# yg838457845/ORB_SLAM2-Chinese-annotation

Measured on AMD Instinct MI355X. Metric: frames/sec (extract+match) at 1241×376, 1000 feat/frame; 1/2/4/8 GPU, higher is better.
Workload: dtype u8; 1 GPU; C4: 1241x376 KITTI-shaped synthetic stream, 1000 feat/frame, SearchByProjection vs 5000-point local map per frame; distinct_frames_per_gpu=8192, frames_per_launch=1024, parallelism=single rank; no collective (one process, one GPU)

## Files before the change

### orb_slam2-chinese-annotation_amd/csrc/extractor_kernels.hip

```cpp
#include <stdlib.h>
#include <type_traits>
#include <algorithm>
#include "orb_device.h"
#include "orb_plan.h"
#include "orb_kernels.h"
#include "orb_pattern_data.h"
#include "../../include/orb_abi.h"

#define PYR_TW 128
#ifndef PYR_IMAGES_PER_WG
#define PYR_IMAGES_PER_WG 16
#endif
#define PYR_TH 32
#define PYR_SROWS 44
#define PYR_SW 44
#define PYR_SROWS_WIDE 64
#define PYR_SW_WIDE 64

__global__ __launch_bounds__(256) void k_pyr_resize_generic(
    const uint8_t* __restrict__ src, long long srcImgPitch, int srcStride, int sw, int sh,
    uint8_t* __restrict__ dst, long long dstImgPitch, int dstStride, int dw, int dh,
    const int* __restrict__ xofs, const int* __restrict__ alpha, const int* __restrict__ yofs,
    const int* __restrict__ beta) {
  const int xs = 4 * (blockIdx.x * 64 + (int)(threadIdx.x & 63));
// ... 789 lines not shown
  h16x2 w3[16];
#pragma unroll
  for (int k = 0; k < 16; ++k)
    w3[k] = __builtin_bit_cast(h16x2, pk_min3_negpair(r[k], r[(k + 1) & 15], r[(k + 2) & 15]));
  h16x2 w9[16];
#pragma unroll
  for (int k = 0; k < 16; ++k)
    w9[k] = __builtin_elementwise_minimum(__builtin_elementwise_minimum(w3[k], w3[(k + 3) & 15]),
                                          w3[(k + 6) & 15]);
  h16x2 m5[6];
#pragma unroll
  for (int k = 0; k < 5; ++k)
    m5[k] = __builtin_elementwise_maximum(__builtin_elementwise_maximum(w9[3 * k], w9[3 * k + 1]),
                                          w9[3 * k + 2]);
  m5[5] = w9[15];
  const h16x2 ma = __builtin_elementwise_maximum(__builtin_elementwise_maximum(m5[0], m5[1]), m5[2]);
  const h16x2 mb = __builtin_elementwise_maximum(__builtin_elementwise_maximum(m5[3], m5[4]), m5[5]);
  h16x2 best = __builtin_elementwise_maximum(ma, mb);
  const _Float16 v = __builtin_bit_cast(_Float16, (uint16_t)c[0]);
  const h16x2 vv = {v, -v};
  best = best + vv;
  const int s = (int)(short)__builtin_bit_cast(uint16_t, __builtin_fmaxf16(best.x, best.y));
  return min(max(s, 0), 255);
}

#ifndef FC_WPE
#define FC_WPE 7
#endif
template <int PT>
__global__ __launch_bounds__(64 * FC_WAVES) __attribute__((amdgpu_waves_per_eu(FC_WPE)))
void k_fast_cells(
    const uint8_t* __restrict__ img0, long long img0Pitch, int img0Stride,
    const uint8_t* __restrict__ arena, long long arenaPitch, OrbPlanDesc plan,
    const OrbCellDesc* __restrict__ cells, uint32_t* __restrict__ cellKeys,
    int32_t* __restrict__ cellCount, int tileElems, int cellBeg, int cellEnd,
    int32_t* __restrict__ errFlag) {
  extern __shared__ __attribute__((aligned(16))) unsigned char smem[];
  const int lane = threadIdx.x & 63;
  const int wave = __builtin_amdgcn_readfirstlane(threadIdx.x >> 6);
  int bx, img;
  xcd_swizzle(bx, img);
  if (errFlag && bx == 0 && threadIdx.x == 0) errFlag[img] = 0;
  uint8_t* tile = smem + wave * fc_wave_bytes(tileElems);
  uint8_t* sc = tile + tileElems;
  uint16_t* queue = (uint16_t*)(sc + tileElems);
  uint16_t* corners = queue + FC_QCAP;
  auto cell_of = [&](int j) { return cellBeg + (bx * FC_CPW + j) * FC_WAVES + wave; };
  uint32_t raw[16], rsh = 0;
  auto issue = [&](const OrbCellDesc& q) {
    const int ql = q.level, qR = q.y1 - q.y0;
    const uint8_t* lvl;
    int pitch;
    if (ql == 0) {
      lvl = img0 + (long long)img * img0Pitch;
      pitch = img0Stride;
    } else {
      lvl = arena + (long long)img * arenaPitch + plan.lv[ql].arenaOff;
      pitch = plan.lv[ql].pitch;
    }
    const ImgRsrc im = img_rsrc(lvl, (uint32_t)((plan.lv[ql].h - 1) * pitch + plan.lv[ql].w));
    const int r = min(lane, max(qR - 1, 0));
    const uint32_t o = (uint32_t)((q.y0 + r) * pitch + q.x0 - FAST_LPAD) + im.sh;
    rsh = o & 3u;
    const uint32_t a0 = o & ~3u;
#pragma unroll
    for (int k = 0; k < 4; ++k) {
      const auto v = __builtin_amdgcn_raw_buffer_load_b128(im.r, (int)(a0 + 16 * k), 0, 0);
      raw[4 * k] = (uint32_t)v[0];
      raw[4 * k + 1] = (uint32_t)v[1];
      raw[4 * k + 2] = (uint32_t)v[2];
      raw[4 * k + 3] = (uint32_t)v[3];
    }
  };
  int ci = cell_of(0);
  if (ci >= cellEnd) return;
  OrbCellDesc ncd = cells[ci];
  issue(ncd);
  for (int jc = 0; jc < FC_CPW && ci < cellEnd; ++jc) {
  const OrbCellDesc cd = ncd;
  const int R = cd.y1 - cd.y0, C = cd.x1 - cd.x0;
  const long long slot = (long long)img * plan.ncells + ci;
  const bool tiny = R < 7 || C < 7;
  const int P = PT ? PT : fc_pitch(C);
  if (!tiny && lane < R) {
    const int nS = P >> 2;
    uint2* dst = reinterpret_cast<uint2*>(tile + lane * P);
#pragma unroll
    for (int k = 0; k < 7; ++k) {
      if (2 * k < nS)
        dst[k] = make_uint2(__builtin_amdgcn_alignbyte(raw[2 * k + 1], raw[2 * k], rsh),
                            __builtin_amdgcn_alignbyte(raw[2 * k + 2], raw[2 * k + 1], rsh));
    }
  }
  {
    uint4* sc16 = reinterpret_cast<uint4*>(tile + tileElems);
    for (int i = lane; i < (tileElems >> 4); i += 64) sc16[i] = make_uint4(0u, 0u, 0u, 0u);
  }
  const int ciNext = jc + 1 < FC_CPW ? cell_of(jc + 1) : cellEnd;
  if (ciNext < cellEnd) {
    ncd = cells[ciNext];
    issue(ncd);
  }
  if (tiny) {
    if (lane == 0) cellCount[slot] = 0;
    ci = ciNext;
    continue;
  }
  const int iw = C - 6, ih = R - 6;
  const int nK = (iw + 7) >> 3;
  const int nvLast = iw - 8 * (nK - 1);
  const int ti = min(max(plan.iniTh, 0), 255), tm = min(max(plan.minTh, 0), 255);
  const float invK = __builtin_amdgcn_rcpf((float)nK), invP = __builtin_amdgcn_rcpf((float)P),
              invW = __builtin_amdgcn_rcpf((float)iw);
  wave_lds_sync();

  int nq = 0, nc = 0;
  auto flush = [&](int t, bool fresh) {
    for (int j0 = 0; j0 < nq; j0 += 64) {
      const int j = j0 + lane;
      bool corner = false;
      int off = 0;
      if (j < nq) {
        off = queue[j];
        int m;
        if (fresh) {
          m = fast_score_u8<(PT != 0)>(tile, off, P);
          sc[off] = (uint8_t)m;
        } else {
          m = sc[off];
          if (m == 0) {
            m = fast_score_u8<(PT != 0)>(tile, off, P);
            sc[off] = (uint8_t)m;
          }
        }
        corner = m > t && m >= 2;
      }
      const unsigned long long bal = __ballot(corner);
      const int pos = nc + (int)__builtin_amdgcn_mbcnt_hi((uint32_t)(bal >> 32),
                                                          __builtin_amdgcn_mbcnt_lo((uint32_t)bal, 0u));
      if (corner && pos < FC_CCAP) corners[pos] = (uint16_t)off;
      nc += __popcll(bal);
    }
    nq = 0;
  };
  auto fast_pass = [&](int t, bool fresh) {
    h16x2 T;
    T.x = T.y = __builtin_bit_cast(_Float16, (uint16_t)(t + 1));
    const int nG = ih * nK;
    const int rr0 = (int)(((float)lane + 0.5f) * invK);
    int k = lane - rr0 * nK;
    int off = (rr0 + 3) * P + 8 + 8 * k;
    const int rInc = (int)(64.5f * invK), kInc = 64 - rInc * nK;
    const int dOff = rInc * P + 8 * kInc, wrapOff = P - 8 * nK;
    for (int g0 = 0; g0 < nG; g0 += 64) {
      const bool valid = g0 + lane < nG;
      const bool last = k == nK - 1;
      const int o = valid ? off : 3 * P + 8;
      {
      const uint2* rw = reinterpret_cast<const uint2*>(tile + o);
      const uint2 A = rw[-1], B = rw[0], Cc = rw[1];
      const uint2 Uu = *reinterpret_cast<const uint2*>(tile + o + 3 * P);
      const uint2 Dd = *reinterpret_cast<const uint2*>(tile + o - 3 * P);
      const uint32_t q4_0 = byte_pair(B.y, B.x, 3, 4);
      const uint32_t V[4] = {byte_pair(B.y, B.x, 0, 1), byte_pair(B.y, B.x, 2, 3),
                             byte_pair(Cc.x, B.y, 0, 1), byte_pair(Cc.x, B.y, 2, 3)};
      const uint32_t Q4[4] = {q4_0, byte_pair(Cc.x, B.y, 1, 2), byte_pair(Cc.x, B.y, 3, 4),
                              byte_pair(Cc.y, Cc.x, 1, 2)};
      const uint32_t Q0[4] = {byte_pair(Uu.y, Uu.x, 0, 1), byte_pair(Uu.y, Uu.x, 2, 3),
                              byte_pair(Uu.y, Uu.x, 4, 5), byte_pair(Uu.y, Uu.x, 6, 7)};
      const uint32_t Q8[4] = {byte_pair(Dd.y, Dd.x, 0, 1), byte_pair(Dd.y, Dd.x, 2, 3),
                              byte_pair(Dd.y, Dd.x, 4, 5), byte_pair(Dd.y, Dd.x, 6, 7)};
      const uint32_t Q12[4] = {byte_pair(A.y, A.x, 5, 6), byte_pair(B.x, A.y, 3, 4),
                               byte_pair(B.x, A.y, 5, 6), q4_0};
      uint32_t rp[4];
#pragma unroll
      for (int i = 0; i < 4; ++i) rp[i] = pretest_pair(V[i], Q0[i], Q4[i], Q8[i], Q12[i], T);
      const uint32_t X = __builtin_amdgcn_perm(rp[1], rp[0], 0x07050301u);
      const uint32_t Y = __builtin_amdgcn_perm(rp[3], rp[2], 0x07050301u);
      const uint32_t fails = ((X >> 7) & 0x01010101u) | ((Y >> 3) & 0x10101010u);
      uint32_t mk = ~((fails * 0x01020408u) >> 24) &
                    (valid ? (last ? (1u << nvLast) - 1u : 0xFFu) : 0u);
      const int cnt = __builtin_popcount(mk);
      int incl = wave_incl_scan(cnt);
      __asm__ volatile("" : "+v"(incl));
      int pos = nq + incl - cnt;
      while (mk) {
        const int j = __builtin_ctz(mk);
        mk &= mk - 1u;
        queue[pos++] = (uint16_t)(off + j);
      }
      nq += __builtin_amdgcn_readlane(incl, 63);
      }
      k += kInc;
      off += dOff;
      if (k >= nK) {
        k -= nK;
        off += wrapOff;
      }
      if (nq > FC_QCAP - 512 || g0 + 64 >= nG) {
        wave_lds_sync();
        flush(t, fresh);
        wave_lds_sync();
      }
    }
  };
  uint32_t* out = cellKeys + slot * plan.keyCap;
  auto nms_emit = [&](int t) -> int {
    const bool dense = nc > FC_CCAP;
    const int nItems = dense ? ih * iw : nc;
    const uint32_t kx0 = (uint32_t)(cd.x0 + 3), ky0 = (uint32_t)(cd.y0 + 3);
    int nOut = 0;
    for (int j0 = 0; j0 < nItems; j0 += 64) {
      const int j = j0 + lane;
      bool ok = false;
      int x = 0, y = 0, m = 0;
      if (j < nItems) {
        int off;
        if (dense) {
          y = (int)(((float)j + 0.5f) * invW);
          x = j - y * iw;
          off = (y + 3) * P + (x + 8);
        } else {
          off = corners[j];
          const int ry = (int)(((float)off + 0.5f) * invP);
          y = ry - 3;
          x = off - ry * P - 8;
        }
        int oq = off - P - 1;
        if (PT) __asm__ volatile("" : "+v"(oq));
        const uint8_t* cq = sc + oq;
        m = cq[P + 1];
        const int nb[8] = {cq[0], cq[1], cq[2], cq[P], cq[P + 2], cq[2 * P], cq[2 * P + 1],
                           cq[2 * P + 2]};
        ok = m > t && m >= 2;
#pragma unroll
        for (int k = 0; k < 8; ++k) ok = ok && !(nb[k] > t && nb[k] >= m);
      }
      const unsigned long long bal = __ballot(ok);
      const int pos = nOut + (int)__builtin_amdgcn_mbcnt_hi((uint32_t)(bal >> 32),
                                                            __builtin_amdgcn_mbcnt_lo((uint32_t)bal, 0u));
      if (ok) out[pos] = pack_key(kx0 + x, ky0 + y, m - 1);
      nOut += __popcll(bal);
    }
    return nOut;
  };
  fast_pass(ti, true);
  int n = nms_emit(ti);
  if (n == 0 && tm != ti) {
    nc = 0;
    fast_pass(tm, false);
    n = nms_emit(tm);
  }
  if (lane == 0) cellCount[slot] = n;
  ci = ciNext;
  wave_lds_sync();
  }
}

struct OctNode {
  int16_t x0, y0, x1, y1;
  int cnt;
  int seq;
};

__device__ __forceinline__ int oct_quad(uint32_t key, const OctNode& n) {
  const int kx = key_x(key) - 16, ky = key_y(key) - 16;
  const int mx = n.x0 + ((n.x1 - n.x0 + 1) >> 1);
  const int my = n.y0 + ((n.y1 - n.y0 + 1) >> 1);
  return (kx < mx ? 0 : 1) + (ky < my ? 0 : 2);
}

__device__ __forceinline__ OctNode oct_child(const OctNode& p, int q, int cnt, int seq) {
  const int mx = p.x0 + ((p.x1 - p.x0 + 1) >> 1);
  const int my = p.y0 + ((p.y1 - p.y0 + 1) >> 1);
  OctNode c;
  c.x0 = (int16_t)((q & 1) ? mx : p.x0);
  c.x1 = (int16_t)((q & 1) ? p.x1 : mx);
  c.y0 = (int16_t)((q & 2) ? my : p.y0);
  c.y1 = (int16_t)((q & 2) ? p.y1 : my);
  c.cnt = cnt;
  c.seq = seq;
  return c;
}

__device__ int block_scan_array(int* a, int n, int* tmp) {
  const int T = blockDim.x, t = threadIdx.x;
// ... 1191 lines not shown
    const int yl = std::min(y0 + PYR_TH - 1, h2 - 1);
    const int Y0 = y0 == 0 ? 0 : std::min(std::max(yo2[y0], 0), h1 - 1);
    const int ownY = y0 + PYR_TH >= h2 ? h1 : std::min(std::max(yo2[y0 + PYR_TH], 0), h1 - 1);
    const int Y1e = std::max(std::min(std::max(yo2[yl] + 1, 0), h1 - 1) + 1, ownY);
    if (ownY < Y0 || Y1e - Y0 > PYR2_R1R) return 0;
    const int r0a = std::min(std::max(yo1[Y0], 0), h0 - 1);
    const int r0b = std::min(std::max(yo1[Y1e - 1] + 1, 0), h0 - 1);
    if (r0b - r0a + 1 > PYR2_S0R) return 0;
  }
  return 1;
}

size_t orb_k_fast_band_lds(int bandElems) {
  const size_t bitBytes = 4 * (size_t)(((bandElems >> 5) + 4) & ~1);
  return (size_t)bandElems * 3 + FAST_QCAP * 2 + FAST_CORNERS * 2 + 2 * bitBytes +
         2 * (size_t)((bandElems / 7 + 15) & ~7) + 2 * ((size_t)bandElems / 28 + 8);
}

hipError_t orb_k_fast_band(const uint8_t* img0, long long img0Pitch, int img0Stride,
                           const uint8_t* arena, long long arenaPitch, const OrbPlanDesc* plan,
                           const OrbBandDesc* bands, int nbands, const OrbCellDesc* cells,
                           uint32_t* cellKeys, int32_t* cellCount, int32_t* errFlag, int nimg,
                           hipStream_t s) {
  const size_t lds = orb_k_fast_band_lds(plan->maxBandBytes);
  const int perWg = nimg <= 2 ? 1 : 2;
  if ((size_t)plan->maxBandBytes > (size_t)4 * FAST_LOADS * 256) return hipErrorInvalidValue;
  dim3 grid((nbands + perWg - 1) / perWg, nimg), block(256);
  hipLaunchKernelGGL(k_fast_band, grid, block, lds, s, img0, img0Pitch, img0Stride, arena,
                     arenaPitch, *plan, bands, cells, nbands, cellKeys, cellCount, errFlag);
  return hipGetLastError();
}

bool orb_k_fast_cells_fits(const OrbPlanDesc* plan) {
  return plan->maxCellRows <= 64 && ((plan->maxCellCols + 20) & ~7) <= 56;
}

size_t orb_k_fast_cells_lds(int maxRows, int maxCols) {
  return (size_t)FC_WAVES * fc_wave_bytes(fc_tile_elems(maxRows, maxCols));
}

hipError_t orb_k_fast_cells(const uint8_t* img0, long long img0Pitch, int img0Stride,
                            const uint8_t* arena, long long arenaPitch, const OrbPlanDesc* plan,
                            const OrbCellDesc* cells, uint32_t* cellKeys, int32_t* cellCount,
                            int32_t* errFlag, int cellBeg, int cellEnd, int nimg, hipStream_t s) {
  if (cellEnd <= cellBeg) return hipSuccess;
  if (!orb_k_fast_cells_fits(plan)) return hipErrorInvalidValue;
  int mr = 7, mc = 7;
  for (int l = 0; l < plan->nlevels; ++l)
    if (plan->lv[l].cellBeg < cellEnd && plan->lv[l].cellEnd > cellBeg) {
      mr = std::max(mr, plan->lv[l].cellMaxRows);
      mc = std::max(mc, plan->lv[l].cellMaxCols);
    }
  const int tileElems = fc_tile_elems(mr, mc);
  const size_t lds = orb_k_fast_cells_lds(mr, mc);
  const bool p56 = fc_pitch(mc) == FC_CONST_PITCH;
  const void* fn = p56 ? (const void*)k_fast_cells<FC_CONST_PITCH> : (const void*)k_fast_cells<0>;
  if (lds > 65536) {
    hipError_t e = hipFuncSetAttribute(fn, hipFuncAttributeMaxDynamicSharedMemorySize, (int)lds);
    if (e != hipSuccess) return e;
  }
  const int n = cellEnd - cellBeg;
  dim3 grid((n + FC_WAVES * FC_CPW - 1) / (FC_WAVES * FC_CPW), nimg), block(64 * FC_WAVES);
  if (p56)
    hipLaunchKernelGGL(k_fast_cells<FC_CONST_PITCH>, grid, block, lds, s, img0, img0Pitch, img0Stride, arena,
                       arenaPitch, *plan, cells, cellKeys, cellCount, tileElems, cellBeg, cellEnd,
                       errFlag);
  else
    hipLaunchKernelGGL(k_fast_cells<0>, grid, block, lds, s, img0, img0Pitch, img0Stride, arena,
                       arenaPitch, *plan, cells, cellKeys, cellCount, tileElems, cellBeg, cellEnd,
                       errFlag);
  return hipGetLastError();
}

size_t orb_k_octree_lds(int nodeCapMax, int maxCellsPerLevel, int ldsKeyCap) {
  int n2 = 1;
  while (n2 < nodeCapMax) n2 <<= 1;
  size_t b = (size_t)n2 * 8 + 2 * (size_t)nodeCapMax * sizeof(OctNode) + (size_t)nodeCapMax * 16 +
             4 * (size_t)nodeCapMax * 4 + (size_t)((maxCellsPerLevel + 3) & ~3) * 4;
  b += (size_t)ldsKeyCap * 4 + (size_t)ldsKeyCap * 2;
  return b;
}

size_t orb_k_octree_node_bytes(int nodeCapMax, int maxCellsPerLevel) {
  return orb_k_octree_lds(nodeCapMax, maxCellsPerLevel, 0);
}

hipError_t orb_k_octree(const OrbPlanDesc* plan, const int32_t* cellCount,
                        const uint32_t* cellKeys, uint32_t* gKeys, uint16_t* gNid, int ldsKeyCap,
                        int nodeCapMax, int maxCellsPerLevel, uint32_t* outKeys,
                        int32_t* outCount, int32_t* errFlag, int levelBeg, int levelEnd, int nimg,
                        uint8_t* gNodes, long long nodeStride, hipStream_t s) {
  if (levelEnd <= levelBeg || nimg <= 0) return hipSuccess;
  const size_t lds = gNodes ? (size_t)ldsKeyCap * 6
                            : orb_k_octree_lds(nodeCapMax, maxCellsPerLevel, ldsKeyCap);
  const bool reg = nimg <= 16;
  const bool gn = gNodes != nullptr;
  const void* fn = reg ? (gn ? (const void*)k_octree<true, true> : (const void*)k_octree<true, false>)
                       : (gn ? (const void*)k_octree<false, true> : (const void*)k_octree<false, false>);
  if (lds > 65536) {
    hipError_t e = hipFuncSetAttribute(fn, hipFuncAttributeMaxDynamicSharedMemorySize, (int)lds);
    if (e != hipSuccess) return e;
  }
// ... 62 lines not shown
```

### orb_slam2-chinese-annotation_amd/csrc/orb_kernels.h

```cpp
#pragma once
#include <hip/hip_runtime.h>
#include <stddef.h>
#include <stdint.h>

#include "../../include/orb_abi.h"
#include "orb_kernel_params.h"
#include "orb_plan.h"

extern "C" {
hipError_t orb_k_copy_pinned(void* dst, const void* src, size_t bytes, hipStream_t s);
hipError_t orb_k_copy_to_pinned(void* dst, const void* src, size_t bytes, hipStream_t s);
hipError_t orb_k_upload_constants(hipStream_t s);
hipError_t orb_k_upload_umax(const int* umax16, hipStream_t s);
hipError_t orb_k_pyr_resize(const uint8_t* src, long long srcImgPitch, int srcStride, int sw,
                            int sh, uint8_t* dst, long long dstImgPitch, int dstStride, int dw,
                            int dh, const int* xofs, const void* alpha, const int* yofs,
                            const void* beta, int mode, int nimg, hipStream_t s);
hipError_t orb_k_pyr_resize2(const uint8_t* src, long long srcImgPitch, int srcStride, int w0,
                             int h0, uint8_t* mid, long long midImgPitch, int midStride, int w1,
                             int h1, const int* xo1, const void* al1, const int* yo1,
                             const void* be1, uint8_t* dst, long long dstImgPitch, int dstStride,
                             int w2, int h2, const int* xo2, const void* al2, const int* yo2,
                             const void* be2, int nimg, hipStream_t s);
int orb_k_pyr_resize2_fits(int w0, int h0, int w1, int h1, const int* xo1, const int* yo1, int w2,
                           int h2, const int* xo2, const int* yo2);
size_t orb_k_fast_band_lds(int bandElems);
hipError_t orb_k_fast_band(const uint8_t* img0, long long img0Pitch, int img0Stride,
                           const uint8_t* arena, long long arenaPitch, const OrbPlanDesc* plan,
                           const OrbBandDesc* bands, int nbands, const OrbCellDesc* cells,
                           uint32_t* cellKeys, int32_t* cellCount, int32_t* errFlag, int nimg,
                           hipStream_t s);
bool orb_k_fast_cells_fits(const OrbPlanDesc* plan);
size_t orb_k_fast_cells_lds(int maxRows, int maxCols);
hipError_t orb_k_fast_cells(const uint8_t* img0, long long img0Pitch, int img0Stride,
                            const uint8_t* arena, long long arenaPitch, const OrbPlanDesc* plan,
                            const OrbCellDesc* cells, uint32_t* cellKeys, int32_t* cellCount,
                            int32_t* errFlag, int cellBeg, int cellEnd, int nimg, hipStream_t s);
size_t orb_k_octree_lds(int nodeCapMax, int maxCellsPerLevel, int ldsKeyCap);
size_t orb_k_octree_node_bytes(int nodeCapMax, int maxCellsPerLevel);
hipError_t orb_k_octree(const OrbPlanDesc* plan, const int32_t* cellCount,
                        const uint32_t* cellKeys, uint32_t* gKeys, uint16_t* gNid, int ldsKeyCap,
                        int nodeCapMax, int maxCellsPerLevel, uint32_t* outKeys,
                        int32_t* outCount, int32_t* errFlag, int levelBeg, int levelEnd, int nimg,
                        uint8_t* gNodes, long long nodeStride, hipStream_t s);
hipError_t orb_k_blur_levels(const uint8_t* img0, long long img0Pitch, int img0Stride,
                             const uint8_t* arena, long long arenaPitch, const OrbPlanDesc* plan,
                             const OrbTileDesc* tiles, uint8_t* blur, long long blurPitch,
                             int nimg, hipStream_t s);
hipError_t orb_k_orient_desc(const uint8_t* img0, long long img0Pitch, int img0Stride,
                             const uint8_t* arena, long long arenaPitch, const OrbPlanDesc* plan,
                             const uint32_t* outKeys, const int32_t* outCount,
                             const int32_t* errFlag, orb_keypoint_t* kps, uint8_t* desc,
                             int capacity, int32_t* counts, int nimg, int levelBeg,
                             int levelEnd, hipStream_t s);

hipError_t orb_k_hamming(const uint8_t* a, const uint8_t* b, int n, int32_t* out, hipStream_t s);
hipError_t orb_k_grid_build(const orb_keypoint_t* keys, const int32_t* nkeys, int kpStride,
                            float minX, float minY, float invW, float invH, int32_t* cellStart,
                            int32_t* cellIdx, int nproblems, hipStream_t s);
hipError_t orb_k_grid_build_staged(const orb_keypoint_t* keys, const int32_t* nkeys,
                                   const uint8_t* locked, const float* uright, int kpStride,
                                   float minX, float minY, float invW, float invH,
                                   int32_t* cellStart, int32_t* cellIdx, void* staged,
                                   int nproblems, hipStream_t s);
int orb_k_grid_stage_max(void);
hipError_t orb_k_proj_candidates(const orb_keypoint_t* keys, const uint8_t* desc,
                                 const float* uright, const uint8_t* locked, int kpStride,
                                 const int32_t* nkeys, const orb_mp_track_t* mps,
                                 const uint8_t* mpDesc, const int32_t* nmps, int mpStride,
// ... 167 lines not shown
```

### orb_slam2-chinese-annotation_amd/csrc/orb_plan.h

```cpp
#pragma once
#include <stdint.h>

#ifndef ORB_MAX_LEVELS
#define ORB_MAX_LEVELS 16
#endif

struct OrbLevelDesc {
  int w, h;
  int pitch;
  int blurPitch;
  long long arenaOff;
  long long blurOff;
  int cellBeg, cellEnd;
  int quota;
  int nodeCap;
  int outOff;
  int nIni;
  float hX;
  int Wr, Hr;
  float scale;
  float sizeF;
  int rtabX, rtabY;
  int xmax;
  int resizeMode;
  int tileBeg;
  int cellMaxRows, cellMaxCols;
  int resize2;
};

#define ORB_RESIZE_NARROW 0
#define ORB_RESIZE_WIDE 1
#define ORB_RESIZE_GENERIC 2

struct OrbPlanDesc {
  int nlevels;
  int ncells;
  int keyCap;
  int slotsPerImage;
  int iniTh, minTh;
  int maxCellRows, maxCellCols;
  int srcW, srcH;
  int nBlurTiles;
  int nBands;
  int maxBandBytes;
  OrbLevelDesc lv[ORB_MAX_LEVELS];
};

struct OrbCellDesc {
  int16_t level, y0, y1, x0, x1, _pad;
};

struct OrbBandDesc {
  int16_t level, y0, y1, x0, x1, nCells;
  int32_t cellBeg;
};
#ifndef ORB_OCTREE_LDS_KB
#define ORB_OCTREE_LDS_KB 52
#endif
#define ORB_BAND_BYTES 6656

struct OrbTileDesc {
  int16_t level, x0, y0, _pad;
};
#define ORB_BLUR_TW 128
#define ORB_BLUR_TH 32
```

### orb_slam2-chinese-annotation_amd/csrc/runtime.cpp

```cpp
#include "runtime_common.h"
#include "orb_synth.h"

static void compute_tables(orb_extractor* h) {
  const int L = h->nlevels;
  h->scale.assign(L, 0.f);
  h->sigma2.assign(L, 0.f);
  h->scale[0] = 1.0f;
  h->sigma2[0] = 1.0f;
  for (int i = 1; i < L; ++i) {
    h->scale[i] = (float)((double)h->scale[i - 1] * h->scaleFactor);
    h->sigma2[i] = h->scale[i] * h->scale[i];
  }
  h->invScale.resize(L);
  h->invSigma2.resize(L);
  for (int i = 0; i < L; ++i) {
    h->invScale[i] = 1.0f / h->scale[i];
    h->invSigma2[i] = 1.0f / h->sigma2[i];
  }
  h->quota.assign(L, 0);
  const float factor = (float)(1.0f / h->scaleFactor);
  float nDesired = (float)h->nfeatures * (1 - factor) /
                   (1 - (float)pow((double)factor, (double)L));
  int sum = 0;
  for (int l = 0; l < L - 1; ++l) {
// ... 51 lines not shown
      for (int x0 = 0; x0 < d.w; x0 += ORB_BLUR_TW) {
        OrbTileDesc t;
        t.level = (int16_t)l;
        t.x0 = (int16_t)x0;
        t.y0 = (int16_t)y0;
        t._pad = 0;
        tiles.push_back(t);
      }
    d.scale = h->scale[l];
    d.sizeF = (float)(int)(31 * h->scale[l]);
    d.quota = h->quota[l];
    const int minBX = 16, minBY = 16, maxBX = d.w - 16, maxBY = d.h - 16;
    const float width = (float)(maxBX - minBX), height = (float)(maxBY - minBY);
    const int nCols = (int)(width / 30.f), nRows = (int)(height / 30.f);
    const int wCell = nCols > 0 ? (int)ceilf(width / nCols) : 0;
    const int hCell = nRows > 0 ? (int)ceilf(height / nRows) : 0;
    d.cellBeg = (int)cells.size();
    for (int i = 0; i < nRows && nCols > 0; ++i) {
      const float iniY = (float)(minBY + i * hCell);
      float maxY = iniY + hCell + 6;
      if (iniY >= maxBY - 3) continue;
      if (maxY > maxBY) maxY = (float)maxBY;
      for (int j = 0; j < nCols; ++j) {
        const float iniX = (float)(minBX + j * wCell);
        float maxX = iniX + wCell + 6;
        if (iniX >= maxBX - 6) continue;
        if (maxX > maxBX) maxX = (float)maxBX;
        OrbCellDesc c;
        c.level = (int16_t)l;
        c.y0 = (int16_t)(int)iniY;
        c.y1 = (int16_t)(int)maxY;
        c.x0 = (int16_t)(int)iniX;
        c.x1 = (int16_t)(int)maxX;
        c._pad = 0;
        cells.push_back(c);
        const int rows = c.y1 - c.y0, cols = c.x1 - c.x0;
        maxRows = std::max(maxRows, rows);
        maxCols = std::max(maxCols, cols);
        d.cellMaxRows = std::max(d.cellMaxRows, rows);
        d.cellMaxCols = std::max(d.cellMaxCols, cols);
        if (rows >= 7 && cols >= 7)
          keyCap = std::max(keyCap, ((rows - 6 + 1) / 2) * ((cols - 6 + 1) / 2));
      }
    }
    d.cellEnd = (int)cells.size();
    for (int c = d.cellBeg; c < d.cellEnd;) {
      OrbBandDesc b;
      b.level = (int16_t)l;
      b.y0 = cells[c].y0;
      b.y1 = cells[c].y1;
      b.x0 = cells[c].x0;
      b.x1 = cells[c].x1;
      b.cellBeg = c;
      int e = c + 1;
      while (e < d.cellEnd && cells[e].y0 == b.y0 && e - c < 64) {
        const int x1 = std::max<int>(b.x1, cells[e].x1);
        if ((b.y1 - b.y0) * ((x1 - b.x0 + 20) & ~7) > bandBudget) break;
        b.x1 = (int16_t)x1;
        ++e;
      }
      b.nCells = (int16_t)(e - c);
      if (b.y1 - b.y0 - 6 > 64) return ORB_EINVAL;
      for (int k = c; k < e; ++k)
        if (cells[k].x1 - cells[k].x0 - 6 > 64) return ORB_EINVAL;
      maxBandBytes = std::max(maxBandBytes, (b.y1 - b.y0) * ((b.x1 - b.x0 + 20) & ~7));
      bands.push_back(b);
      c = e;
// ... 31 lines not shown
        }
        for (int y0 = 0; y0 < d.h; y0 += 32) {
          const int yl = std::min(y0 + 31, d.h - 1);
          const int syA = std::min(std::max(yo[y0], 0), sh - 1);
          const int syB = std::min(std::max(yo[yl] + 1, 0), sh - 1);
          if (syB - syA + 1 > SR) return false;
        }
        return true;
      };
      const bool narrowOk = (double)sw / d.w <= 1.25 && (double)sh / d.h <= 1.25;
      const bool bounded = orb_resize_weights_bounded(&rtab[d.rtabX + d.w], d.w) &&
                           orb_resize_weights_bounded(&rtab[d.rtabY + d.h], d.h);
      d.resizeMode = !bounded                        ? ORB_RESIZE_GENERIC
                     : narrowOk && tiles_fit(44, 44) ? ORB_RESIZE_NARROW
                     : tiles_fit(64, 64)             ? ORB_RESIZE_WIDE
                                                     : ORB_RESIZE_GENERIC;
    }
  }
  int nResize = 0;
  for (int l = 1; l < L;) {
    OrbLevelDesc& d = P.lv[l];
    d.resize2 = 0;
    if (l + 1 < L && d.resizeMode == ORB_RESIZE_NARROW &&
        P.lv[l + 1].resizeMode == ORB_RESIZE_NARROW) {
      const OrbLevelDesc& e = P.lv[l + 1];
      d.resize2 = orb_k_pyr_resize2_fits(P.lv[l - 1].w, P.lv[l - 1].h, d.w, d.h, &rtab[d.rtabX],
                                         &rtab[d.rtabY], e.w, e.h, &rtab[e.rtabX], &rtab[e.rtabY]);
    }
    l += d.resize2 ? 2 : 1;
    ++nResize;
  }
  if (orb_k_fast_band_lds(maxBandBytes) > 64 * 1024) return ORB_EINVAL;
  P.ncells = (int)cells.size();
  P.nBlurTiles = (int)tiles.size();
  P.nBands = (int)bands.size();
  P.maxBandBytes = maxBandBytes;
  P.keyCap = keyCap;
  P.slotsPerImage = slots;
  P.maxCellRows = maxRows;
  P.maxCellCols = maxCols;
  const size_t nodeBytes = orb_k_octree_lds(nodeCapMax, maxCellsPerLevel, 0);
  const size_t budget = (size_t)ORB_OCTREE_LDS_KB * 1024;
  const bool octGlobal = nodeBytes > 128 * 1024;
  const size_t ldsNodes = octGlobal ? 0 : nodeBytes;
  int ldsKeyCap = ldsNodes < budget ? (int)((budget - ldsNodes) / 6) : 0;
  ldsKeyCap &= ~7;
  if (ldsNodes + (size_t)ldsKeyCap * 6 > 160 * 1024) return ORB_EINVAL;

  hipSetDevice(h->device);
  if (must_wait(h->lastStream, h->stream)) HIP_TRY(hipStreamWaitEvent(h->stream, h->evBatch, 0));
  orb_status_t st = h->dCells.ensure(cells.size() * sizeof(OrbCellDesc));
  if (st) return st;
  st = h->dRtab.ensure(std::max<size_t>(rtab.size(), 1) * 4);
  if (st) return st;
  st = h->dTiles.ensure(tiles.size() * sizeof(OrbTileDesc));
  if (st) return st;
  st = h->dBands.ensure(bands.size() * sizeof(OrbBandDesc));
  if (st) return st;
  HIP_TRY(hipMemcpyAsync(h->dBands.p, bands.data(), bands.size() * sizeof(OrbBandDesc),
                         hipMemcpyHostToDevice, h->stream));
  HIP_TRY(hipMemcpyAsync(h->dTiles.p, tiles.data(), tiles.size() * sizeof(OrbTileDesc),
                         hipMemcpyHostToDevice, h->stream));
  HIP_TRY(hipMemcpyAsync(h->dCells.p, cells.data(), cells.size() * sizeof(OrbCellDesc),
                         hipMemcpyHostToDevice, h->stream));
  if (!rtab.empty())
    HIP_TRY(hipMemcpyAsync(h->dRtab.p, rtab.data(), rtab.size() * 4, hipMemcpyHostToDevice,
                           h->stream));
  HIP_TRY(stream_wait(h->stream));
  h->lastStream = nullptr;
  h->plan = P;
  h->cells.swap(cells);
  h->arenaBytes = (arena + 255) & ~255LL;
  h->blurBytes = (blurArena + 255) & ~255LL;
  h->maxCellsPerLevel = maxCellsPerLevel;
  h->nodeCapMax = nodeCapMax;
  h->ldsKeyCap = ldsKeyCap;
  h->octNodeBytes = octGlobal ? (long long)((nodeBytes + 255) & ~(size_t)255) : 0;
  h->planW = W;
  h->planH = H;
  h->nResizePairs = nResize;
  h->prof.launchesPerCall[0] = nResize;
  h->batchCap = 0;
  return ORB_OK;
}

static orb_status_t ensure_batch(orb_extractor* h, int B) {
  if (B <= h->batchCap) return ORB_OK;
  const OrbPlanDesc& P = h->plan;
  const size_t cellSlots = (size_t)B * P.ncells * P.keyCap;
  orb_status_t st;
  if ((st = h->dArena.ensure((size_t)B * h->arenaBytes))) return st;
  if ((st = h->dCellKeys.ensure(cellSlots * 4))) return st;
  if ((st = h->dGKeys.ensure(cellSlots * 4))) return st;
  if ((st = h->dGNid.ensure(cellSlots * 2))) return st;
  if ((st = h->dCellCount.ensure((size_t)B * P.ncells * 4))) return st;
  if ((st = h->dOutKeys.ensure((size_t)B * P.slotsPerImage * 4))) return st;
  if ((st = h->dOutCount.ensure((size_t)B * P.nlevels * 4))) return st;
  if ((st = h->dErr.ensure((size_t)B * 4))) return st;
  if (h->octNodeBytes &&
      (st = h->dOctNodes.ensure((size_t)B * P.nlevels * (size_t)h->octNodeBytes)))
    return st;
  h->batchCap = B;
  return ORB_OK;
}
// ... 7 lines not shown
#ifndef FAST_SIDE_LEVELS
#define FAST_SIDE_LEVELS 2
#endif
#ifndef FAST_L0_INLINE
#define FAST_L0_INLINE 0
#endif

static orb_status_t run_batch(orb_extractor* h, const uint8_t* d_images, int B, size_t stride,
                              size_t imgPitch, orb_keypoint_t* d_kps, uint8_t* d_desc,
                              int capacity, int32_t* d_counts, hipStream_t s,
                              bool capturing = false) {
  const OrbPlanDesc& P = h->plan;
  const int32_t* rt = h->dRtab.as<int32_t>();
  uint8_t* arena = h->dArena.as<uint8_t>();
  const long long ap = h->arenaBytes;
  std::shared_lock<std::shared_mutex> sideUse(g_sideUse);
  if (g_sideReleased) return ORB_EDEVICE;
  hipStream_t side = h->stream2;
  capturing = capturing || stream_capturing(s);
  {
    if (capturing) {
      if (!h->privSide &&
          hipStreamCreateWithPriority(&h->privSide, hipStreamNonBlocking, least_stream_prio()) != hipSuccess) {
        h->privSide = nullptr;
        return ORB_EDEVICE;
      }
      side = h->privSide;
    }
  }
  StageProfiler& pf = h->prof;
  std::vector<hipEvent_t>* ev = pf.begin_call();
  PROF_REC(ev, pf.t0(ev), s);
  if (P.ncells == 0) HIP_TRY(hipMemsetAsync(h->dErr.p, 0, (size_t)B * 4, s));
  const bool useBands = B < FAST_CELLS_MIN_BATCH || !orb_k_fast_cells_fits(&P);
  pf.names[2] = useBands ? "k_fast_band" : "k_fast_cells";
  auto fast = [&](int cb, int ce, hipStream_t st) -> hipError_t {
    return orb_k_fast_cells(d_images, (long long)imgPitch, (int)stride, arena, ap, &P,
                            h->dCells.as<OrbCellDesc>(), h->dCellKeys.as<uint32_t>(),
                            h->dCellCount.as<int32_t>(), h->dErr.as<int32_t>(), cb, ce, B, st);
  };
  const int l0End = P.lv[0].cellEnd;
  const bool l0Side = !useBands && !FAST_L0_INLINE && !(ev && pf.serial) && l0End > 0 && P.nlevels > 1;
  const int sideLevels = l0Side ? std::min(FAST_SIDE_LEVELS, P.nlevels - 1) : 0;
  const int sideEnd = sideLevels > 0 ? P.lv[sideLevels].cellEnd : l0End;
  if (l0Side) {
    HIP_TRY(hipEventRecord(h->evL0Fork, s));
    HIP_TRY(hipStreamWaitEvent(side, h->evL0Fork, 0));
    PROF_REC(ev, pf.b(ev, 5), side);
    HIP_TRY(fast(0, l0End, side));
    PROF_REC(ev, pf.e(ev, 5), side);
    if (sideLevels == 0) HIP_TRY(hipEventRecord(h->evL0Join, side));
  } else if (ev) {
    pf.not_run(5);
  }
  PROF_REC(ev, pf.b(ev, 0), s);
  const bool pairs = B <= PYR_PAIR_MAX_IMAGES;
  h->prof.launchesPerCall[0] = pairs ? h->nResizePairs : P.nlevels - 1;
  for (int l = 1; l < P.nlevels; ++l) {
    const OrbLevelDesc& d = P.lv[l];
    const OrbLevelDesc& sd = P.lv[l - 1];
    const uint8_t* src = l == 1 ? d_images : arena + sd.arenaOff;
    const long long srcPitch = l == 1 ? (long long)imgPitch : ap;
    const int srcStride = l == 1 ? (int)stride : sd.pitch;
    const bool pair = pairs && d.resize2;
    const int top = pair ? l + 1 : l;
    if (pair) {
      const OrbLevelDesc& e = P.lv[l + 1];
      HIP_TRY(orb_k_pyr_resize2(src, srcPitch, srcStride, sd.w, sd.h, arena + d.arenaOff, ap, d.pitch,
                                d.w, d.h, rt + d.rtabX, rt + d.rtabX + d.w, rt + d.rtabY,
                                rt + d.rtabY + d.h, arena + e.arenaOff, ap, e.pitch, e.w, e.h,
                                rt + e.rtabX, rt + e.rtabX + e.w, rt + e.rtabY, rt + e.rtabY + e.h,
                                B, s));
// ... 2470 lines not shown
```

### orb_slam2-chinese-annotation_amd/csrc/runtime_common.h

```cpp
#ifndef ORB_RUNTIME_COMMON_H
#define ORB_RUNTIME_COMMON_H

#include <hip/hip_runtime.h>
#include <math.h>
#include <stdint.h>
#include <stdio.h>
#include <stdlib.h>
#include <string.h>

#include <algorithm>
#include <array>
#include <chrono>
#include <mutex>
#include <shared_mutex>
#include <cmath>
#include <unordered_map>
#include <vector>

#include "../../include/orb_abi.h"
#include "orb_kernels.h"
#include "orb_resize_tables.h"

namespace {

// ... 212 lines not shown
  return (size_t)width;
}

static inline orb_status_t upload(DevBuf& b, const void* src, size_t n, hipStream_t s) {
  orb_status_t st = b.ensure(std::max<size_t>(n, 16));
  if (st) return st;
  if (n) HIP_TRY(hipMemcpyAsync(b.p, src, n, hipMemcpyHostToDevice, s));
  return ORB_OK;
}

}

struct orb_extractor {
  int device = 0;
  int nfeatures = 0, nlevels = 0, iniTh = 0, minTh = 0;
  float scaleFactorF = 1.2f;
  double scaleFactor = 1.2;
  std::vector<float> scale, invScale, sigma2, invSigma2;
  std::vector<int> quota;
  int umax[16];
  hipStream_t stream = nullptr;
  hipStream_t stream2 = nullptr;
  hipStream_t privSide = nullptr;
  hipEvent_t evL0Fork = nullptr, evL0Join = nullptr;
  hipEvent_t evLvl = nullptr;
  hipEvent_t evBatch = nullptr;
  hipStream_t lastStream = nullptr;
  bool ownStream = false;
  std::mutex mu;

  int planW = -1, planH = -1;
  OrbPlanDesc plan;
  std::vector<OrbCellDesc> cells;
  long long arenaBytes = 0, blurBytes = 0;
  int maxCellsPerLevel = 0, nodeCapMax = 0, ldsKeyCap = 0;
  int nResizePairs = 0;
  DevBuf dCells, dRtab, dTiles, dBands;

  int batchCap = 0;
  DevBuf dBlur;
  DevBuf dArena, dCellKeys, dCellCount, dGKeys, dGNid, dOutKeys, dOutCount, dErr;
  DevBuf dOctNodes;
  long long octNodeBytes = 0;
  DevBuf dImg, dOne;
  HostBuf hImg, hOut, hLvl;
  HostBuf hPyr;
  bool pyrReadback = false, hPyrValid = false;
  int oneCap = 0;
  bool lastSingle = false;
  hipGraphExec_t oneExec = nullptr;
  std::vector<const void*> oneKey;
  int lastW = 0, lastH = 0;
  size_t lastImgStride = 0;
  const uint8_t* lastImg0 = nullptr;
  size_t lastImg0Pitch = 0;
  int lastImg0Stride = 0;

  StageProfiler prof;
};

enum MatcherSlot {
  PP_FRAME0 = 0, PP_FRAME1 = 4,
  PP_MPS = 8, PP_MPDESC, PP_VALID, PP_SKIP, PP_ANGLE, PP_URIGHT, PP_RECS, PP_TOPK, PP_NCAND,
  PP_BEST, PP_LOCKED, PP_KPMATCH, PP_COUNT, PP_BEST12, PP_BEST21, PP_MUTUAL, SX_COUNT,
  BW_DESC1 = 0, BW_ANGLE1, BW_MP1, BW_BAD1, BW_IDS1, BW_OFFS1, BW_FEATS1,
  BW_DESC2, BW_ANGLE2, BW_MP2, BW_BAD2, BW_IDS2, BW_OFFS2, BW_FEATS2, BW_MATCH, BW_ACC, BW_COUNT,
// ... 74 lines not shown
```

Measured before the change: 368,500 frames/s.

## Precompute per-cell-class constants on host and use magic-number division in FAST cells

Adds a host-built table of cell classes (level, size), each holding precomputed pitch, masks, loop increments and fixed-point reciprocal multipliers. The FAST cell kernel now reads these instead of recomputing divisions and rcp-based quotients per cell. It also caches the level buffer resource across cells of the same level, zeroes only the used part of the score tile, uses a dot4 for the fail mask and a max-reduction for NMS. In exchange it adds host-side exactness checks and a fallback to the band path when the magic divisions are not exact.

```diff
diff --git a/orb_slam2-chinese-annotation_amd/csrc/extractor_kernels.hip b/orb_slam2-chinese-annotation_amd/csrc/extractor_kernels.hip
--- a/orb_slam2-chinese-annotation_amd/csrc/extractor_kernels.hip
+++ b/orb_slam2-chinese-annotation_amd/csrc/extractor_kernels.hip
@@ -845,10 +845,11 @@
 void k_fast_cells(
     const uint8_t* __restrict__ img0, long long img0Pitch, int img0Stride,
     const uint8_t* __restrict__ arena, long long arenaPitch, OrbPlanDesc plan,
-    const OrbCellDesc* __restrict__ cells, uint32_t* __restrict__ cellKeys,
-    int32_t* __restrict__ cellCount, int tileElems, int cellBeg, int cellEnd,
-    int32_t* __restrict__ errFlag) {
+    const OrbCellDesc* __restrict__ cells, const OrbCellClass* __restrict__ classes,
+    uint32_t* __restrict__ cellKeys, int32_t* __restrict__ cellCount, int tileElems, int cellBeg,
+    int cellEnd, int32_t* __restrict__ errFlag) {
   extern __shared__ __attribute__((aligned(16))) unsigned char smem[];
+  static_assert(FC_CONST_PITCH == ORB_FC_CONST_PITCH, "the class table's mP48 is this pitch's");
   const int lane = threadIdx.x & 63;
   const int wave = __builtin_amdgcn_readfirstlane(threadIdx.x >> 6);
   int bx, img;
@@ -859,21 +860,30 @@
   uint16_t* queue = (uint16_t*)(sc + tileElems);
   uint16_t* corners = queue + FC_QCAP;
   auto cell_of = [&](int j) { return cellBeg + (bx * FC_CPW + j) * FC_WAVES + wave; };
+  const uint32_t* cellW = reinterpret_cast<const uint32_t*>(cells);
   uint32_t raw[16], rsh = 0;
-  auto issue = [&](const OrbCellDesc& q) {
-    const int ql = q.level, qR = q.y1 - q.y0;
-    const uint8_t* lvl;
-    int pitch;
-    if (ql == 0) {
-      lvl = img0 + (long long)img * img0Pitch;
-      pitch = img0Stride;
-    } else {
-      lvl = arena + (long long)img * arenaPitch + plan.lv[ql].arenaOff;
-      pitch = plan.lv[ql].pitch;
-    }
-    const ImgRsrc im = img_rsrc(lvl, (uint32_t)((plan.lv[ql].h - 1) * pitch + plan.lv[ql].w));
-    const int r = min(lane, max(qR - 1, 0));
-    const uint32_t o = (uint32_t)((q.y0 + r) * pitch + q.x0 - FAST_LPAD) + im.sh;
+  ImgRsrc im = {};
+  int lvPitch = 0, lvCur = -1;
+  auto issue = [&](uint32_t w0, uint32_t w1, uint32_t w2) {
+    const int ql = (int)(w0 & 0xFFFFu), qy0 = (int)(w0 >> 16), qy1 = (int)(w1 & 0xFFFFu),
+              qx0 = (int)(w1 >> 16);
+    if (ql != lvCur) {
+      const OrbCellClass& qc = classes[w2 >> 16];
+      const uint8_t* lvl;
+      if (ql == 0) {
+        lvl = img0 + (long long)img * img0Pitch;
+        lvPitch = img0Stride;
+      } else {
+        lvl = arena + (long long)img * arenaPitch +
+              (long long)(((unsigned long long)qc.arenaHi << 32) | qc.arenaLo);
+        lvPitch = qc.pitch;
+      }
+      im = img_rsrc(lvl, (uint32_t)(qc.h1 * lvPitch + qc.w));
+      lvCur = ql;
+    }
+    const int r = min(lane, max(qy1 - qy0 - 1, 0));
+    const uint32_t o = __umul24((uint32_t)(qy0 + r), (uint32_t)lvPitch) +
+                       ((uint32_t)(qx0 - FAST_LPAD) + im.sh);
     rsh = o & 3u;
     const uint32_t a0 = o & ~3u;
 #pragma unroll
@@ -887,17 +897,28 @@
   };
   int ci = cell_of(0);
   if (ci >= cellEnd) return;
-  OrbCellDesc ncd = cells[ci];
-  issue(ncd);
+  uint32_t nw0 = cellW[3 * ci], nw1 = cellW[3 * ci + 1], nw2 = cellW[3 * ci + 2];
+  issue(nw0, nw1, nw2);
+  uint32_t* const imgKeys = cellKeys + (long long)img * plan.ncells * plan.keyCap;
+  int32_t* const imgCount = cellCount + (long long)img * plan.ncells;
+  const int ti = min(max(plan.iniTh, 0), 255), tm = min(max(plan.minTh, 0), 255);
   for (int jc = 0; jc < FC_CPW && ci < cellEnd; ++jc) {
-  const OrbCellDesc cd = ncd;
-  const int R = cd.y1 - cd.y0, C = cd.x1 - cd.x0;
-  const long long slot = (long long)img * plan.ncells + ci;
-  const bool tiny = R < 7 || C < 7;
-  const int P = PT ? PT : fc_pitch(C);
+  const uint32_t cw0 = nw0, cw1 = nw1;
+  const OrbCellClass& kc = classes[nw2 >> 16];
+  const int R = kc.R;
+  const bool tiny = kc.tiny != 0;
+  const int P = PT ? PT : kc.P;
+  const int iw = kc.iw, ih = kc.ih, nK = kc.nK, lastMask = kc.lastMask, nG = kc.nG, kInc = kc.kInc;
+  const int dOff = PT ? kc.dOff48 : kc.dOff, wrapOff = PT ? kc.wrapOff48 : kc.wrapOff;
+  const uint32_t mP = PT ? kc.mP48 : kc.mP, mW = kc.mW;
+  const int rr0 = (int)(__umul24((uint32_t)lane, kc.mK) >> ORB_QUOT_SHIFT);
+  const int k0 = lane - (int)__umul24((uint32_t)rr0, (uint32_t)nK);
+  const int off0 = (int)__umul24((uint32_t)(rr0 + 3), (uint32_t)P) + 8 + 8 * k0;
+  const int slotOff = ci;
   if (!tiny && lane < R) {
     const int nS = P >> 2;
-    uint2* dst = reinterpret_cast<uint2*>(tile + lane * P);
+    const uint32_t rowOff = __umul24((uint32_t)lane, (uint32_t)P);
+    uint2* dst = reinterpret_cast<uint2*>(tile + rowOff);
 #pragma unroll
     for (int k = 0; k < 7; ++k) {
       if (2 * k < nS)
@@ -905,26 +926,23 @@
                             __builtin_amdgcn_alignbyte(raw[2 * k + 2], raw[2 * k + 1], rsh));
     }
   }
-  {
-    uint4* sc16 = reinterpret_cast<uint4*>(tile + tileElems);
-    for (int i = lane; i < (tileElems >> 4); i += 64) sc16[i] = make_uint4(0u, 0u, 0u, 0u);
+  if (!tiny) {
+    uint4* sc16 = reinterpret_cast<uint4*>(sc + 2 * P);
+    const int n16 = ((R - 4) * P + 15) >> 4;
+    for (int i = lane; i < n16; i += 64) sc16[i] = make_uint4(0u, 0u, 0u, 0u);
   }
   const int ciNext = jc + 1 < FC_CPW ? cell_of(jc + 1) : cellEnd;
   if (ciNext < cellEnd) {
-    ncd = cells[ciNext];
-    issue(ncd);
+    nw0 = cellW[3 * ciNext];
+    nw1 = cellW[3 * ciNext + 1];
+    nw2 = cellW[3 * ciNext + 2];
+    issue(nw0, nw1, nw2);
   }
   if (tiny) {
-    if (lane == 0) cellCount[slot] = 0;
+    if (lane == 0) imgCount[slotOff] = 0;
     ci = ciNext;
     continue;
   }
-  const int iw = C - 6, ih = R - 6;
-  const int nK = (iw + 7) >> 3;
-  const int nvLast = iw - 8 * (nK - 1);
-  const int ti = min(max(plan.iniTh, 0), 255), tm = min(max(plan.minTh, 0), 255);
-  const float invK = __builtin_amdgcn_rcpf((float)nK), invP = __builtin_amdgcn_rcpf((float)P),
-              invW = __builtin_amdgcn_rcpf((float)iw);
   wave_lds_sync();
 
   int nq = 0, nc = 0;
@@ -959,12 +977,7 @@
   auto fast_pass = [&](int t, bool fresh) {
     h16x2 T;
     T.x = T.y = __builtin_bit_cast(_Float16, (uint16_t)(t + 1));
-    const int nG = ih * nK;
-    const int rr0 = (int)(((float)lane + 0.5f) * invK);
-    int k = lane - rr0 * nK;
-    int off = (rr0 + 3) * P + 8 + 8 * k;
-    const int rInc = (int)(64.5f * invK), kInc = 64 - rInc * nK;
-    const int dOff = rInc * P + 8 * kInc, wrapOff = P - 8 * nK;
+    int k = k0, off = off0;
     for (int g0 = 0; g0 < nG; g0 += 64) {
       const bool valid = g0 + lane < nG;
       const bool last = k == nK - 1;
@@ -991,8 +1004,8 @@
       const uint32_t X = __builtin_amdgcn_perm(rp[1], rp[0], 0x07050301u);
       const uint32_t Y = __builtin_amdgcn_perm(rp[3], rp[2], 0x07050301u);
       const uint32_t fails = ((X >> 7) & 0x01010101u) | ((Y >> 3) & 0x10101010u);
-      uint32_t mk = ~((fails * 0x01020408u) >> 24) &
-                    (valid ? (last ? (1u << nvLast) - 1u : 0xFFu) : 0u);
+      uint32_t mk = ~__builtin_amdgcn_udot4(fails, 0x08040201u, 0u, false) &
+                    (valid ? (last ? (uint32_t)lastMask : 0xFFu) : 0u);
       const int cnt = __builtin_popcount(mk);
       int incl = wave_incl_scan(cnt);
       __asm__ volatile("" : "+v"(incl));
@@ -1017,11 +1030,11 @@
       }
     }
   };
-  uint32_t* out = cellKeys + slot * plan.keyCap;
+  uint32_t* out = imgKeys + slotOff * plan.keyCap;
   auto nms_emit = [&](int t) -> int {
     const bool dense = nc > FC_CCAP;
     const int nItems = dense ? ih * iw : nc;
-    const uint32_t kx0 = (uint32_t)(cd.x0 + 3), ky0 = (uint32_t)(cd.y0 + 3);
+    const uint32_t kx0 = (cw1 >> 16) + 3u, ky0 = (cw0 >> 16) + 3u;
     int nOut = 0;
     for (int j0 = 0; j0 < nItems; j0 += 64) {
       const int j = j0 + lane;
@@ -1030,14 +1043,14 @@
       if (j < nItems) {
         int off;
         if (dense) {
-          y = (int)(((float)j + 0.5f) * invW);
-          x = j - y * iw;
-          off = (y + 3) * P + (x + 8);
+          y = (int)(__umul24((uint32_t)j, mW) >> ORB_QUOT_SHIFT);
+          x = j - (int)__umul24((uint32_t)y, (uint32_t)iw);
+          off = (int)__umul24((uint32_t)(y + 3), (uint32_t)P) + (x + 8);
         } else {
           off = corners[j];
-          const int ry = (int)(((float)off + 0.5f) * invP);
+          const int ry = (int)(__umul24((uint32_t)off, mP) >> ORB_QUOT_SHIFT);
           y = ry - 3;
-          x = off - ry * P - 8;
+          x = off - 8 + __mul24(ry, -P);
         }
         int oq = off - P - 1;
         if (PT) __asm__ volatile("" : "+v"(oq));
@@ -1045,9 +1058,10 @@
         m = cq[P + 1];
         const int nb[8] = {cq[0], cq[1], cq[2], cq[P], cq[P + 2], cq[2 * P], cq[2 * P + 1],
                            cq[2 * P + 2]};
-        ok = m > t && m >= 2;
-#pragma unroll
-        for (int k = 0; k < 8; ++k) ok = ok && !(nb[k] > t && nb[k] >= m);
+        int nbMax = nb[0];
+#pragma unroll
+        for (int k = 1; k < 8; ++k) nbMax = max(nbMax, nb[k]);
+        ok = m > t && m >= 2 && nbMax < m;
       }
       const unsigned long long bal = __ballot(ok);
       const int pos = nOut + (int)__builtin_amdgcn_mbcnt_hi((uint32_t)(bal >> 32),
@@ -1064,7 +1078,7 @@
     fast_pass(tm, false);
     n = nms_emit(tm);
   }
-  if (lane == 0) cellCount[slot] = n;
+  if (lane == 0) imgCount[slotOff] = n;
   ci = ciNext;
   wave_lds_sync();
   }
@@ -2322,7 +2336,8 @@
 }
 
 bool orb_k_fast_cells_fits(const OrbPlanDesc* plan) {
-  return plan->maxCellRows <= 64 && ((plan->maxCellCols + 20) & ~7) <= 56;
+  return plan->maxCellRows <= 64 && ((plan->maxCellCols + 20) & ~7) <= 56 &&
+         plan->cellClassesOk && (long long)plan->ncells * plan->keyCap < (1LL << 31);
 }
 
 size_t orb_k_fast_cells_lds(int maxRows, int maxCols) {
@@ -2331,10 +2346,12 @@
 
 hipError_t orb_k_fast_cells(const uint8_t* img0, long long img0Pitch, int img0Stride,
                             const uint8_t* arena, long long arenaPitch, const OrbPlanDesc* plan,
-                            const OrbCellDesc* cells, uint32_t* cellKeys, int32_t* cellCount,
-                            int32_t* errFlag, int cellBeg, int cellEnd, int nimg, hipStream_t s) {
+                            const OrbCellDesc* cells, const OrbCellClass* classes,
+                            uint32_t* cellKeys, int32_t* cellCount, int32_t* errFlag, int cellBeg,
+                            int cellEnd, int nimg, hipStream_t s) {
   if (cellEnd <= cellBeg) return hipSuccess;
-  if (!orb_k_fast_cells_fits(plan)) return hipErrorInvalidValue;
+  if (!orb_k_fast_cells_fits(plan) || img0Stride < 0 || img0Stride >= (1 << 24))
+    return hipErrorInvalidValue;
   int mr = 7, mc = 7;
   for (int l = 0; l < plan->nlevels; ++l)
     if (plan->lv[l].cellBeg < cellEnd && plan->lv[l].cellEnd > cellBeg) {
@@ -2353,11 +2370,11 @@
   dim3 grid((n + FC_WAVES * FC_CPW - 1) / (FC_WAVES * FC_CPW), nimg), block(64 * FC_WAVES);
   if (p56)
     hipLaunchKernelGGL(k_fast_cells<FC_CONST_PITCH>, grid, block, lds, s, img0, img0Pitch, img0Stride, arena,
-                       arenaPitch, *plan, cells, cellKeys, cellCount, tileElems, cellBeg, cellEnd,
+                       arenaPitch, *plan, cells, classes, cellKeys, cellCount, tileElems, cellBeg, cellEnd,
                        errFlag);
   else
     hipLaunchKernelGGL(k_fast_cells<0>, grid, block, lds, s, img0, img0Pitch, img0Stride, arena,
-                       arenaPitch, *plan, cells, cellKeys, cellCount, tileElems, cellBeg, cellEnd,
+                       arenaPitch, *plan, cells, classes, cellKeys, cellCount, tileElems, cellBeg, cellEnd,
                        errFlag);
   return hipGetLastError();
 }
diff --git a/orb_slam2-chinese-annotation_amd/csrc/orb_kernels.h b/orb_slam2-chinese-annotation_amd/csrc/orb_kernels.h
--- a/orb_slam2-chinese-annotation_amd/csrc/orb_kernels.h
+++ b/orb_slam2-chinese-annotation_amd/csrc/orb_kernels.h
@@ -34,7 +34,8 @@
 size_t orb_k_fast_cells_lds(int maxRows, int maxCols);
 hipError_t orb_k_fast_cells(const uint8_t* img0, long long img0Pitch, int img0Stride,
                             const uint8_t* arena, long long arenaPitch, const OrbPlanDesc* plan,
-                            const OrbCellDesc* cells, uint32_t* cellKeys, int32_t* cellCount,
+                            const OrbCellDesc* cells, const OrbCellClass* classes,
+                            uint32_t* cellKeys, int32_t* cellCount,
                             int32_t* errFlag, int cellBeg, int cellEnd, int nimg, hipStream_t s);
 size_t orb_k_octree_lds(int nodeCapMax, int maxCellsPerLevel, int ldsKeyCap);
 size_t orb_k_octree_node_bytes(int nodeCapMax, int maxCellsPerLevel);
diff --git a/orb_slam2-chinese-annotation_amd/csrc/orb_plan.h b/orb_slam2-chinese-annotation_amd/csrc/orb_plan.h
--- a/orb_slam2-chinese-annotation_amd/csrc/orb_plan.h
+++ b/orb_slam2-chinese-annotation_amd/csrc/orb_plan.h
@@ -43,12 +43,109 @@
   int nBlurTiles;
   int nBands;
   int maxBandBytes;
+  int nCellClasses;
+  int cellClassesOk;
   OrbLevelDesc lv[ORB_MAX_LEVELS];
 };
 
 struct OrbCellDesc {
-  int16_t level, y0, y1, x0, x1, _pad;
+  int16_t level, y0, y1, x0, x1, cls;
 };
+
+#define ORB_QUOT_SHIFT 18
+#define ORB_FC_PITCH(C) (((C) + 12) & ~7)
+#define ORB_FC_CONST_PITCH 48
+struct OrbCellClass {
+  int32_t level, pitch, w, h1;
+  uint32_t arenaLo, arenaHi;
+  int32_t R, C;
+  int32_t tiny;
+  int32_t P;
+  int32_t iw, ih;
+  int32_t nK;
+  int32_t lastMask;
+  int32_t nG;
+  int32_t kInc;
+  int32_t dOff, wrapOff;
+  uint32_t mP;
+  int32_t dOff48, wrapOff48;
+  uint32_t mP48;
+  uint32_t mK, mW;
+};
+
+static inline uint32_t orb_quot_magic(int d) {
+  return d > 0 ? (uint32_t)(((1u << ORB_QUOT_SHIFT) + (uint32_t)d - 1u) / (uint32_t)d) : 0u;
+}
+
+static inline void orb_cell_class_fill(OrbCellClass* k, const OrbLevelDesc* lv, int level, int R,
+                                       int C) {
+  *k = OrbCellClass();
+  k->level = level;
+  k->pitch = level ? lv->pitch : 0;
+  k->w = lv->w;
+  k->h1 = lv->h - 1;
+  k->arenaLo = (uint32_t)((unsigned long long)lv->arenaOff & 0xFFFFFFFFull);
+  k->arenaHi = (uint32_t)((unsigned long long)lv->arenaOff >> 32);
+  k->R = R;
+  k->C = C;
+  k->tiny = R < 7 || C < 7;
+  if (k->tiny) return;
+  k->P = ORB_FC_PITCH(C);
+  k->iw = C - 6;
+  k->ih = R - 6;
+  k->nK = (k->iw + 7) >> 3;
+  k->lastMask = (1 << (k->iw - 8 * (k->nK - 1))) - 1;
+  k->nG = k->ih * k->nK;
+  const int rInc = 64 / k->nK;
+  k->kInc = 64 - rInc * k->nK;
+  k->dOff = rInc * k->P + 8 * k->kInc;
+  k->wrapOff = k->P - 8 * k->nK;
+  k->mP = orb_quot_magic(k->P);
+  k->dOff48 = rInc * ORB_FC_CONST_PITCH + 8 * k->kInc;
+  k->wrapOff48 = ORB_FC_CONST_PITCH - 8 * k->nK;
+  k->mP48 = orb_quot_magic(ORB_FC_CONST_PITCH);
+  k->mK = orb_quot_magic(k->nK);
+  k->mW = orb_quot_magic(k->iw);
+}
+
+static inline bool orb_quot_exact(uint32_t m, int d, int n) {
+  if (d <= 0 || n <= 0 || m >= (1u << 24) || n > (1 << 24)) return false;
+  if ((unsigned long long)(n - 1) * m >= (1ull << 32)) return false;
+  for (int x = 0; x < n; ++x)
+    if (((uint32_t)x * m) >> ORB_QUOT_SHIFT != (uint32_t)(x / d)) return false;
+  return true;
+}
+
+static inline bool orb_cell_class_ok(const OrbCellClass* k) {
+  if (k->pitch < 0 || k->pitch >= (1 << 24) || k->R > 64) return false;
+  if (k->tiny) return true;
+  if (k->P > 56) return false;
+  if (!orb_quot_exact(k->mK, k->nK, 64)) return false;
+  if (!orb_quot_exact(k->mP, k->P, k->R * k->P)) return false;
+  if (k->P <= ORB_FC_CONST_PITCH &&
+      !orb_quot_exact(k->mP48, ORB_FC_CONST_PITCH, k->R * ORB_FC_CONST_PITCH))
+    return false;
+  return orb_quot_exact(k->mW, k->iw, k->ih * k->iw);
+}
+
+static inline int orb_build_cell_classes(const OrbPlanDesc* plan, OrbCellDesc* cells, int ncells,
+                                         OrbCellClass* out, int cap) {
+  int n = 0;
+  for (int i = 0; i < ncells; ++i) {
+    OrbCellDesc& c = cells[i];
+    const int R = c.y1 - c.y0, C = c.x1 - c.x0;
+    int j = n - 1;
+    while (j >= 0 && !(out[j].level == c.level && out[j].R == R && out[j].C == C)) --j;
+    if (j < 0) {
+      if (n == cap) return -1;
+      orb_cell_class_fill(&out[n], &plan->lv[c.level], c.level, R, C);
+      j = n++;
+    }
+    c.cls = (int16_t)j;
+  }
+  return n;
+}
+#define ORB_MAX_CELL_CLASSES (8 * ORB_MAX_LEVELS)
 
 struct OrbBandDesc {
   int16_t level, y0, y1, x0, x1, nCells;
diff --git a/orb_slam2-chinese-annotation_amd/csrc/runtime.cpp b/orb_slam2-chinese-annotation_amd/csrc/runtime.cpp
--- a/orb_slam2-chinese-annotation_amd/csrc/runtime.cpp
+++ b/orb_slam2-chinese-annotation_amd/csrc/runtime.cpp
@@ -107,7 +107,7 @@
         c.y1 = (int16_t)(int)maxY;
         c.x0 = (int16_t)(int)iniX;
         c.x1 = (int16_t)(int)maxX;
-        c._pad = 0;
+        c.cls = 0;
         cells.push_back(c);
         const int rows = c.y1 - c.y0, cols = c.x1 - c.x0;
         maxRows = std::max(maxRows, rows);
@@ -205,6 +205,13 @@
   }
   if (orb_k_fast_band_lds(maxBandBytes) > 64 * 1024) return ORB_EINVAL;
   P.ncells = (int)cells.size();
+  std::vector<OrbCellClass> classes(ORB_MAX_CELL_CLASSES);
+  const int nClasses =
+      orb_build_cell_classes(&P, cells.data(), P.ncells, classes.data(), ORB_MAX_CELL_CLASSES);
+  classes.resize(std::max(nClasses, 0));
+  P.nCellClasses = (int)classes.size();
+  P.cellClassesOk = nClasses >= 0;
+  for (const OrbCellClass& k : classes) P.cellClassesOk = P.cellClassesOk && orb_cell_class_ok(&k);
   P.nBlurTiles = (int)tiles.size();
   P.nBands = (int)bands.size();
   P.maxBandBytes = maxBandBytes;
@@ -222,7 +229,8 @@
 
   hipSetDevice(h->device);
   if (must_wait(h->lastStream, h->stream)) HIP_TRY(hipStreamWaitEvent(h->stream, h->evBatch, 0));
-  orb_status_t st = h->dCells.ensure(cells.size() * sizeof(OrbCellDesc));
+  const size_t classOff = (cells.size() * sizeof(OrbCellDesc) + 15) & ~(size_t)15;
+  orb_status_t st = h->dCells.ensure(classOff + std::max<size_t>(classes.size(), 1) * sizeof(OrbCellClass));
   if (st) return st;
   st = h->dRtab.ensure(std::max<size_t>(rtab.size(), 1) * 4);
   if (st) return st;
@@ -236,6 +244,9 @@
                          hipMemcpyHostToDevice, h->stream));
   HIP_TRY(hipMemcpyAsync(h->dCells.p, cells.data(), cells.size() * sizeof(OrbCellDesc),
                          hipMemcpyHostToDevice, h->stream));
+  if (!classes.empty())
+    HIP_TRY(hipMemcpyAsync((char*)h->dCells.p + classOff, classes.data(),
+                           classes.size() * sizeof(OrbCellClass), hipMemcpyHostToDevice, h->stream));
   if (!rtab.empty())
     HIP_TRY(hipMemcpyAsync(h->dRtab.p, rtab.data(), rtab.size() * 4, hipMemcpyHostToDevice,
                            h->stream));
@@ -243,6 +254,7 @@
   h->lastStream = nullptr;
   h->plan = P;
   h->cells.swap(cells);
+  h->cellClassOff = classOff;
   h->arenaBytes = (arena + 255) & ~255LL;
   h->blurBytes = (blurArena + 255) & ~255LL;
   h->maxCellsPerLevel = maxCellsPerLevel;
@@ -316,12 +328,14 @@
   std::vector<hipEvent_t>* ev = pf.begin_call();
   PROF_REC(ev, pf.t0(ev), s);
   if (P.ncells == 0) HIP_TRY(hipMemsetAsync(h->dErr.p, 0, (size_t)B * 4, s));
-  const bool useBands = B < FAST_CELLS_MIN_BATCH || !orb_k_fast_cells_fits(&P);
+  const bool useBands = B < FAST_CELLS_MIN_BATCH || !orb_k_fast_cells_fits(&P) || stride >= (1 << 24);
   pf.names[2] = useBands ? "k_fast_band" : "k_fast_cells";
   auto fast = [&](int cb, int ce, hipStream_t st) -> hipError_t {
     return orb_k_fast_cells(d_images, (long long)imgPitch, (int)stride, arena, ap, &P,
-                            h->dCells.as<OrbCellDesc>(), h->dCellKeys.as<uint32_t>(),
-                            h->dCellCount.as<int32_t>(), h->dErr.as<int32_t>(), cb, ce, B, st);
+                            h->dCells.as<OrbCellDesc>(),
+                            (const OrbCellClass*)((const char*)h->dCells.p + h->cellClassOff),
+                            h->dCellKeys.as<uint32_t>(), h->dCellCount.as<int32_t>(),
+                            h->dErr.as<int32_t>(), cb, ce, B, st);
   };
   const int l0End = P.lv[0].cellEnd;
   const bool l0Side = !useBands && !FAST_L0_INLINE && !(ev && pf.serial) && l0End > 0 && P.nlevels > 1;
diff --git a/orb_slam2-chinese-annotation_amd/csrc/runtime_common.h b/orb_slam2-chinese-annotation_amd/csrc/runtime_common.h
--- a/orb_slam2-chinese-annotation_amd/csrc/runtime_common.h
+++ b/orb_slam2-chinese-annotation_amd/csrc/runtime_common.h
@@ -268,6 +268,7 @@
   int planW = -1, planH = -1;
   OrbPlanDesc plan;
   std::vector<OrbCellDesc> cells;
+  size_t cellClassOff = 0;
   long long arenaBytes = 0, blurBytes = 0;
   int maxCellsPerLevel = 0, nodeCapMax = 0, ldsKeyCap = 0;
   int nResizePairs = 0;
```

Result: faster. 378,900 frames/s, median of 6 (+2.8%).
